# OxfordML/GPz

Measured on AMD Instinct MI355X. Metric: objective+gradient evals/sec, higher is better.
Workload: dtype f64

## Files before the change

### gpz_amd/csrc/gpz_options.h

```cpp
#pragma once

struct gpz_options {
    bool no_graph = false;
    bool graph_debug = false;
    long row_tile = 0;
    long cache_cap_mb = -1;
    bool psi32_mfma = false;
    long predict_min_rows_per_block = 4096;
    bool f32_contractions_off = false;
    bool gc_minv_off = false;
    bool gc_dense_phi_off = false;
    bool tgemm_no_split = false;
    bool phi_diag_no_split = false;
    bool pmc_scratch = false;
    bool pmc_prep_scratch = false;
    bool pmc_no_model_cache = false;
    bool round_phi32 = false;
    bool cpsi_off = false;
    bool cpsi4_off = false;
    bool tgemm_int8 = false;
    int syrk_wgs = 0, syrk_s1 = 0, syrk_s2 = 0;
    int mom_nc = 0;
    int small_stagger = 0;
    bool chol_rowinv_off = false;
    bool syrk_small_off = false;
    bool small_tail_off = false;
    int debug_fail_cut = 0;
};

gpz_options gpz_options_load();

const gpz_options &gpz_opts();
struct gpz_opts_scope {
    const gpz_options *prev;
    explicit gpz_opts_scope(const gpz_options *o);
    ~gpz_opts_scope();
    gpz_opts_scope(const gpz_opts_scope &) = delete;
    gpz_opts_scope &operator=(const gpz_opts_scope &) = delete;
};
```

### gpz_amd/csrc/gpz_options.hip

```cpp
#include <stdlib.h>
#include "gpz_options.h"

static const char *env(const char *name) { return getenv(name); }
static bool env_set(const char *name) { return env(name) != nullptr; }
static long env_long(const char *name, long dflt) {
    const char *e = env(name);
    return e ? atol(e) : dflt;
}

gpz_options gpz_options_load() {
    gpz_options o;
    o.no_graph = env_set("GPZ_NO_GRAPH");
    o.graph_debug = env_set("GPZ_GRAPH_DEBUG");
    o.row_tile = env_long("GPZ_ROW_TILE", 0);
    o.cache_cap_mb = env_long("GPZ_CACHE_CAP_MB", -1);
    {
        const char *e = env("GPZ_PSI32_MFMA");
        o.psi32_mfma = e && e[0] == '1';
    }
    o.predict_min_rows_per_block = env_long("GPZ_PREDICT_MIN_ROWS_PER_BLOCK", 4096);
    if (o.predict_min_rows_per_block < 1) o.predict_min_rows_per_block = 1;
#ifdef GPZ_DEV_SWITCHES
    o.f32_contractions_off = env_set("GPZ_F32_CONTRACTIONS_OFF");
    o.gc_minv_off = env_set("GPZ_GC_MINV_OFF");
    o.gc_dense_phi_off = env_set("GPZ_GC_DENSE_PHI_OFF");
    o.tgemm_no_split = env_set("GPZ_TGEMM_NO_SPLIT");
    o.phi_diag_no_split = env_set("GPZ_PHI_DIAG_NO_SPLIT");
    o.pmc_scratch = env_set("GPZ_PMC_SCRATCH");
    o.pmc_prep_scratch = env_set("GPZ_PMC_PREP_SCRATCH");
    o.pmc_no_model_cache = env_set("GPZ_PMC_NO_MODEL_CACHE");
    o.round_phi32 = env_set("GPZ_EXPERIMENT_ROUND_PHI32");
    o.cpsi_off = env_set("GPZ_CPSI_OFF");
    o.cpsi4_off = env_set("GPZ_CPSI4_OFF");
    o.tgemm_int8 = env_set("GPZ_TGEMM_INT8");
    o.syrk_wgs = (int)env_long("GPZ_SYRK_WGS", 0);
    o.syrk_s1 = (int)env_long("GPZ_SYRK_S1", 0);
    o.syrk_s2 = (int)env_long("GPZ_SYRK_S2", 0);
    o.mom_nc = (int)env_long("GPZ_MOM_NC", 0);
    o.debug_fail_cut = (int)env_long("GPZ_DEBUG_FAIL_CUT", 0);
    o.small_tail_off = env_set("GPZ_SMALL_TAIL_OFF");
    o.syrk_small_off = env_set("GPZ_SYRK_SMALL_OFF");
    o.chol_rowinv_off = env_set("GPZ_CHOL_ROWINV_OFF");
    o.small_stagger = (int)env_long("GPZ_SMALL_STAGGER", 0);
#endif
    return o;
}

static thread_local const gpz_options *t_opts = nullptr;
const gpz_options &gpz_opts() {
    if (t_opts) return *t_opts;
    static const gpz_options process = gpz_options_load();
    return process;
}
gpz_opts_scope::gpz_opts_scope(const gpz_options *o) : prev(t_opts) { t_opts = o; }
gpz_opts_scope::~gpz_opts_scope() { t_opts = prev; }
```

### gpz_amd/csrc/k_gemm.hip

```cpp
#include <type_traits>
#include "gpz_dev.h"
#include "gpz_kernels.h"

#ifdef GPZ_GEMM_TRACE
__device__ unsigned long long *g_gemm_trace = nullptr;
#define GPZ_TRACE_MARK(slot)                                                                                              \
    do {                                                                                                                  \
        if (g_gemm_trace && (threadIdx.x & 63) == 0)                                                                      \
            g_gemm_trace[((size_t)item * 8 + (threadIdx.x >> 6)) * 6 + (slot)] = __builtin_amdgcn_s_memtime();       \
    } while (0)
#else
#define GPZ_TRACE_MARK(slot) do { } while (0)
#endif
typedef float f4_t __attribute__((ext_vector_type(4)));
typedef float f2_t __attribute__((ext_vector_type(2)));
#ifndef GPZ_F32_FLUSH
#define GPZ_F32_FLUSH 8
#endif
template <typename OT> struct MfmaOf;
template <> struct MfmaOf<double> {
    typedef d4_t acc_t;
    typedef d2_t pair_t;
    static __device__ __forceinline__ acc_t run(double a, double b, acc_t c) { return MFMA_F64(a, b, c); }
};
template <> struct MfmaOf<float> {
    typedef f4_t acc_t;
    typedef f2_t pair_t;
    static __device__ __forceinline__ acc_t run(float a, float b, acc_t c) { return __builtin_amdgcn_mfma_f32_16x16x4f32(a, b, c, 0, 0, 0); }
};
template <typename OT>
__device__ __forceinline__ typename MfmaOf<OT>::pair_t to_pair(const f2_t v) {
    typename MfmaOf<OT>::pair_t r;
    r.x = (OT)v.x;
    r.y = (OT)v.y;
    return r;
}
template <typename BT> struct Pair2 { typedef d2_t t; };
template <> struct Pair2<float> { typedef f2_t t; };
template <typename OT>
__device__ __forceinline__ typename MfmaOf<OT>::pair_t to_pair(const d2_t v) {
    typename MfmaOf<OT>::pair_t r;
    r.x = (OT)v.x;
    r.y = (OT)v.y;
    return r;
}

template <bool WEIGHTED, int WC, bool DIAGT, typename OT>
__device__ __forceinline__ void syrk_body(const double *__restrict__ Phi, int ld, const double *__restrict__ wgt,
                                          int mp, int i0, int j0, int r_begin, int r_end,
                                          double *__restrict__ out, OT (*sA)[16][LDS_LD128],
                                          OT (*sB)[16][LDS_LD128], OT (*sW)[16]) {
    constexpr int NT = 128 * WC;
    constexpr int NI = 8 / WC;
    constexpr int Q = 1024 / NT;
    constexpr bool diag_tile = DIAGT;
    constexpr bool PRESCALE = WEIGHTED;
    const int tid = threadIdx.x, lane = tid & 63, wave = tid >> 6;
    const int wr = wave / WC, wc = wave % WC;

    constexpr bool F32 = std::is_same<OT, float>::value;
    typedef typename MfmaOf<OT>::acc_t acc_t;
    typedef typename MfmaOf<OT>::pair_t pair_t;
    acc_t acc[4][NI];
    d4_t acc64[F32 ? 4 : 1][F32 ? NI : 1];
#pragma unroll
    for (int a = 0; a < 4; ++a)
#pragma unroll
        for (int b = 0; b < NI; ++b) {
            acc[a][b] = (acc_t){0, 0, 0, 0};
            if (F32) acc64[a][b] = (d4_t){0.0, 0.0, 0.0, 0.0};
        }
    auto flush = [&]() {
        if constexpr (F32) {
#pragma unroll
            for (int a = 0; a < 4; ++a)
#pragma unroll
                for (int b = 0; b < NI; ++b) {
#pragma unroll
                    for (int r = 0; r < 4; ++r) acc64[a][b][r] += (double)acc[a][b][r];
                    acc[a][b] = (acc_t){0, 0, 0, 0};
                }
        }
    };

    d2_t ra[Q], rb[Q];
    double rw = 0.0, rwq[PRESCALE ? Q : 1];
    const int ca = min(i0 + (tid & 63) * 2, mp - 2), cb = min(j0 + (tid & 63) * 2, mp - 2);
    const unsigned voa = (unsigned)(((tid >> 6) * ld + ca) * 8), vob = (unsigned)(((tid >> 6) * ld + cb) * 8);
    const unsigned vow = (unsigned)((PRESCALE ? (tid >> 6) : (tid & 15)) * 8);
    const size_t qsp = (size_t)(NT / 64) * ld * 8, ksp = (size_t)16 * ld * 8;
    const char *pp = reinterpret_cast<const char *>(Phi + (size_t)r_begin * ld);
    const char *pw = reinterpret_cast<const char *>(WEIGHTED ? wgt + r_begin : nullptr);
    auto gload = [&]() {
        unsigned oa = voa, ob = vob, ow = vow;
        asm volatile("" : "+v"(oa), "+v"(ob), "+v"(ow));
#pragma unroll
        for (int q = 0; q < Q; ++q) {
            ra[q] = *reinterpret_cast<const d2_t *>(pp + q * qsp + oa);
            if (!diag_tile) rb[q] = *reinterpret_cast<const d2_t *>(pp + q * qsp + ob);
            if (PRESCALE) rwq[q] = *reinterpret_cast<const double *>(pw + q * (NT / 64) * 8 + ow);
        }
        if (WEIGHTED && !PRESCALE && tid < 16) rw = *reinterpret_cast<const double *>(pw + ow);
        pp += ksp;
        if (WEIGHTED) pw += 16 * 8;
    };
    auto lstore = [&](int buf) {
#pragma unroll
        for (int q = 0; q < Q; ++q) {
            int idx = q * NT + tid;
            int row = idx >> 6, c = (idx & 63) * 2;
            if (diag_tile) *reinterpret_cast<pair_t *>(&sB[buf][row][c]) = to_pair<OT>(ra[q]);
            else *reinterpret_cast<pair_t *>(&sB[buf][row][c]) = to_pair<OT>(rb[q]);
            if (PRESCALE) { ra[q].x *= rwq[q]; ra[q].y *= rwq[q]; }
            *reinterpret_cast<pair_t *>(&sA[buf][row][c]) = to_pair<OT>(ra[q]);
        }
        if (WEIGHTED && !PRESCALE && tid < 16) sW[buf][tid] = (OT)rw;
    };

    const int nstage = (r_end > r_begin) ? (r_end - r_begin) / 16 : 0;
    if (nstage > 0) {
        gload();
        lstore(0);
        if (nstage > 1) gload();
    }
    __syncthreads();
    static_assert(!DIAGT || NI == 2, "diagonal-tile wave roles are written for the 2 x 4 wave grid");
    constexpr int NA = 4, NB = DIAGT ? 5 : NI;
    int dra[5] = {0, 0, 0, 0, 0}, dcb[5] = {0, 0, 0, 0, 0};
    bool has5 = false;
    if (DIAGT) {
        const int wv = __builtin_amdgcn_readfirstlane(wave);
        const unsigned RA[8] = {0x00000u, 0x11111u, 0x22222u, 0x33333u, 0x77000u, 0x66611u, 0x55552u, 0x44444u};
        const unsigned CB[8] = {0x43210u, 0x54321u, 0x65432u, 0x76543u, 0x77765u, 0x77676u, 0x77657u, 0x77654u};
        has5 = wv < 4;
#pragma unroll
        for (int p = 0; p < 5; ++p) {
            dra[p] = (RA[wv] >> (4 * p)) & 15;
            dcb[p] = (CB[wv] >> (4 * p)) & 15;
        }
    }
    auto rdfrag = [&](int cur, int kk, OT (&a)[NA], OT (&b)[NB]) {
        const OT(*tA)[LDS_LD128] = sA[cur];
        const OT(*tB)[LDS_LD128] = sB[cur];
        const int krow = kk * 4 + (lane >> 4);
        if (DIAGT) {
#pragma unroll
            for (int p = 0; p < 4; ++p) a[p] = tA[krow][dra[p] * 16 + (lane & 15)];
#pragma unroll
            for (int p = 0; p < 5; ++p) b[p] = tB[krow][dcb[p] * 16 + (lane & 15)];
        } else {
#pragma unroll
            for (int mi = 0; mi < 4; ++mi) a[mi] = tA[krow][wr * 64 + mi * 16 + (lane & 15)];
#pragma unroll
            for (int ni = 0; ni < NI; ++ni) b[ni] = tB[krow][wc * (16 * NI) + ni * 16 + (lane & 15)];
        }
    };
    auto burst = [&](const OT (&a)[NA], const OT (&b)[NB]) {
        __builtin_amdgcn_s_setprio(1);
        if (DIAGT) {
#pragma unroll
            for (int p = 0; p < 4; ++p) acc[p][0] = MfmaOf<OT>::run(a[p], b[p], acc[p][0]);
            if (has5) acc[0][1] = MfmaOf<OT>::run(a[0], b[DIAGT ? 4 : 0], acc[0][1]);
        } else {
#pragma unroll
            for (int mi = 0; mi < 4; ++mi)
#pragma unroll
                for (int ni = 0; ni < NI; ++ni) acc[mi][ni] = MfmaOf<OT>::run(a[mi], b[ni], acc[mi][ni]);
        }
        __builtin_amdgcn_s_setprio(0);
    };
    OT fa0[NA] = {}, fb0[NB] = {}, fa1[NA] = {}, fb1[NB] = {};
    if (nstage > 0) rdfrag(0, 0, fa0, fb0);
    auto stage = [&](auto curc, int s) {
        constexpr int cur = decltype(curc)::value;
        rdfrag(cur, 1, fa1, fb1);
        __builtin_amdgcn_sched_barrier(0);
        burst(fa0, fb0);
        __builtin_amdgcn_sched_barrier(0);
        rdfrag(cur, 2, fa0, fb0);
        __builtin_amdgcn_sched_barrier(0);
        burst(fa1, fb1);
        __builtin_amdgcn_sched_barrier(0);
        if (s + 1 < nstage) {
            lstore(cur ^ 1);
            if (s + 2 < nstage) gload();
        }
        rdfrag(cur, 3, fa1, fb1);
        __builtin_amdgcn_sched_barrier(0);
        burst(fa0, fb0);
        __builtin_amdgcn_sched_barrier(0);
        __syncthreads();
        if (s + 1 < nstage) rdfrag(cur ^ 1, 0, fa0, fb0);
        __builtin_amdgcn_sched_barrier(0);
        burst(fa1, fb1);
        __builtin_amdgcn_sched_barrier(0);
    };
    int s = 0;
    for (; s + 1 < nstage; s += 2) {
        stage(std::integral_constant<int, 0>{}, s);
        stage(std::integral_constant<int, 1>{}, s + 1);
        if (F32 && ((s + 2) % GPZ_F32_FLUSH) == 0) flush();
    }
    if (s < nstage) stage(std::integral_constant<int, 0>{}, s);
    flush();
    auto res = [&](int mi, int ni, int r) -> double {
        if constexpr (F32) return acc64[mi][ni][r];
        else return acc[mi][ni][r];
    };
    auto crow = [&](int r) -> int { return F32 ? 4 * (lane >> 4) + r : (lane >> 4) + 4 * r; };

    if (DIAGT) {
#pragma unroll
        for (int p = 0; p < 5; ++p) {
            if (p == 4 && !has5) break;
            const int col = j0 + dcb[p] * 16 + (lane & 15);
#pragma unroll
            for (int r = 0; r < 4; ++r) {
                const int row = i0 + dra[p] * 16 + crow(r);
                if (row < mp && col < mp) out[(size_t)row * mp + col] = p < 4 ? res(p, 0, r) : res(0, 1, r);
            }
        }
    } else {
#pragma unroll
        for (int mi = 0; mi < 4; ++mi)
#pragma unroll
            for (int ni = 0; ni < NI; ++ni) {
                const int col = j0 + wc * (16 * NI) + ni * 16 + (lane & 15);
#pragma unroll
                for (int r = 0; r < 4; ++r) {
                    const int row = i0 + wr * 64 + mi * 16 + crow(r);
                    if (row < mp && col < mp) out[(size_t)row * mp + col] = res(mi, ni, r);
                }
            }
    }
}

template <bool WEIGHTED, bool TRI, int WC, typename OT>
__global__ __launch_bounds__(128 * WC, (std::is_same<OT, float>::value ? 2 : WC)) void k_syrk(
    const double *__restrict__ Phi, int ld, const double *__restrict__ wgt, int n_rows, int mp, int ntile, int nsplit,
    int rows_per_split, int nsplit_d, int rows_per_split_d, double *__restrict__ slab) {
    __shared__ OT sA[2][16][LDS_LD128];
    __shared__ OT sB[2][16][LDS_LD128];
    __shared__ OT sW[2][16];

    const int npairs = ntile * (ntile + 1) / 2;
    const int nwg = gridDim.x, xcd = blockIdx.x & 7, qq = nwg >> 3, rr = nwg & 7;
    const int lb = (xcd < rr ? xcd * (qq + 1) : rr * (qq + 1) + (xcd - rr) * qq) + (blockIdx.x >> 3);
    const int noff = npairs - ntile, ndiag = ntile * nsplit_d;
    auto gstart = [&](int g) { return g * noff + g * ndiag / nsplit; };
    int g = (int)((unsigned)lb * (unsigned)nsplit / (unsigned)(noff * nsplit + ndiag));
    g = g > nsplit - 1 ? nsplit - 1 : g;
    while (g > 0 && gstart(g) > lb) --g;
    while (g + 1 < nsplit && gstart(g + 1) <= lb) ++g;
    const int within = lb - gstart(g);
    int ti, tj, split, rps;
    if (within < noff) {
        split = g;
        rps = rows_per_split;
        int rem = within;
        ti = 0;
        while (rem >= ntile - 1 - ti) { rem -= ntile - 1 - ti; ++ti; }
        tj = ti + 1 + rem;
    } else {
        const int q = g * ndiag / nsplit + within - noff;
        split = q / ntile;
        rps = rows_per_split_d;
        ti = tj = q % ntile;
    }
    const bool diag_tile = (ti == tj);
    const int i0 = ti * 128, j0 = tj * 128;

    int r_begin = split * rps;
    int r_end = min(n_rows, r_begin + rps);
    if (TRI) r_begin = max(r_begin, j0 & ~15);
    double *out = slab + (size_t)split * mp * mp;
    if (diag_tile)
        syrk_body<WEIGHTED, WC, true, OT>(Phi, ld, wgt, mp, i0, j0, r_begin, r_end, out, sA, sB, sW);
    else
        syrk_body<WEIGHTED, WC, false, OT>(Phi, ld, wgt, mp, i0, j0, r_begin, r_end, out, sA, sB, sW);
}

__global__ void k_syrk_reduce(const double *__restrict__ slab, int nsplit_off, int nsplit_d, int mp,
                              double *__restrict__ S, int lds, int accumulate) {
    const int j = blockIdx.x * blockDim.x + threadIdx.x;
    const int i = blockIdx.y;
    if (j >= mp || i > j) return;
    const int ti = i >> 7, tj = j >> 7;
    const int nsplit = (ti == tj) ? nsplit_d : nsplit_off;
    const size_t stride = (size_t)mp * mp;
    const double *p = slab + (size_t)i * mp + j;
    double s0 = 0.0, s1 = 0.0, s2 = 0.0, s3 = 0.0;
    int k = 0;
    for (; k + 8 <= nsplit; k += 8) {
        double v[8];
#pragma unroll
        for (int q = 0; q < 8; ++q) v[q] = p[(size_t)(k + q) * stride];
        s0 += v[0]; s1 += v[1]; s2 += v[2]; s3 += v[3];
        s0 += v[4]; s1 += v[5]; s2 += v[6]; s3 += v[7];
    }
    for (; k < nsplit; ++k) s0 += p[(size_t)k * stride];
    const double t = (s0 + s1) + (s2 + s3);
    S[(size_t)i * lds + j] = accumulate ? S[(size_t)i * lds + j] + t : t;
    if (i != j) S[(size_t)j * lds + i] = accumulate ? S[(size_t)j * lds + i] + t : t;
}

template <bool EDGE, int WC, typename OT, typename BT>
__device__ __forceinline__ void tgemm_body(const double *__restrict__ Phi, int ld, const BT *__restrict__ B,
                                           int ldb, double *__restrict__ T, int ldt, int mp, int i0, int j0,
                                           OT (*sA)[128][18], OT (*sB)[16][LDS_LD128],
                                           double *__restrict__ nupart, double *__restrict__ phiw, int m, int mcol,
                                           long n_pad, int ct, int kdim, int ncol16 = 8, int slot = 0, int nslot = 1, int item = 0) {
    constexpr int NT = 128 * WC;
    constexpr int NI = 8 / WC;
    constexpr int Q = 1024 / NT;
    const int tid = threadIdx.x, lane = tid & 63, wave = tid >> 6;
    const int wr = wave / WC, wc = wave % WC;

    typedef typename MfmaOf<OT>::acc_t acc_t;
    typedef typename MfmaOf<OT>::pair_t pair_t;
    acc_t acc[4][NI];
#pragma unroll
    for (int a = 0; a < 4; ++a)
#pragma unroll
        for (int b = 0; b < NI; ++b) acc[a][b] = (acc_t){0, 0, 0, 0};

    typedef typename Pair2<BT>::t bpair_t;
    d2_t ra[Q];
    bpair_t rb[Q];
    const unsigned voa = (unsigned)(((tid >> 3) * ld + (tid & 7) * 2) * 8);
    const unsigned vob = (unsigned)(((tid >> 6) * ldb + min(j0 + (tid & 63) * 2, mp - 2)) * sizeof(BT));
    const size_t qsa = (size_t)(NT / 8) * ld * 8, qsb = (size_t)(NT / 64) * ldb * sizeof(BT), ksb = (size_t)16 * ldb * sizeof(BT);
    const char *pa = reinterpret_cast<const char *>(Phi + (size_t)i0 * ld);
    const char *pb = reinterpret_cast<const char *>(B);
    auto gload = [&]() {
        unsigned oa = voa, ob = vob;
        asm volatile("" : "+v"(oa), "+v"(ob));
#pragma unroll
        for (int q = 0; q < Q; ++q) {
            ra[q] = *reinterpret_cast<const d2_t *>(pa + q * qsa + oa);
            rb[q] = *reinterpret_cast<const bpair_t *>(pb + q * qsb + ob);
        }
        pa += 16 * 8;
        pb += ksb;
    };
    auto lstore = [&](int buf) {
#pragma unroll
        for (int q = 0; q < Q; ++q) {
            int idx = q * NT + tid;
            int arow = idx >> 3, ac = (idx & 7) * 2;
            *reinterpret_cast<pair_t *>(&sA[buf][arow][ac]) = to_pair<OT>(ra[q]);
            int row = idx >> 6, c = (idx & 63) * 2;
            *reinterpret_cast<pair_t *>(&sB[buf][row][c]) = to_pair<OT>(rb[q]);
        }
    };

    int nvalid = NI;
    if (EDGE) {
        nvalid = (mp - j0 + 15) / 16;
        nvalid = nvalid < 0 ? 0 : (nvalid > ncol16 ? ncol16 : nvalid);
        nvalid = __builtin_amdgcn_readfirstlane(nvalid);
    }
    static_assert(!EDGE || 4 * NI == 8, "the row-strip deal keeps its eight accumulators in acc[4][2]");
    constexpr int NFA = EDGE ? 1 : 4, NFB = EDGE ? 8 : NI;

    const int nstage = kdim / 16;
    gload();
    lstore(0);
    if (nstage > 1) gload();
    __syncthreads();
    auto rdfrag = [&](int cur, int kk, OT (&a)[NFA], OT (&b)[NFB]) {
        const int kc = kk * 4 + (lane >> 4);
        if (EDGE) {
            a[0] = sA[cur][wave * 16 + (lane & 15)][kc];
#pragma unroll
            for (int p = 0; p < NFB; ++p) b[p] = sB[cur][kc][p * 16 + (lane & 15)];
        } else {
#pragma unroll
            for (int mi = 0; mi < NFA; ++mi) a[mi] = sA[cur][wr * 64 + mi * 16 + (lane & 15)][kc];
#pragma unroll
            for (int ni = 0; ni < NI; ++ni) b[ni] = sB[cur][kc][wc * (16 * NI) + ni * 16 + (lane & 15)];
        }
    };
    auto burst = [&](const OT (&a)[NFA], const OT (&b)[NFB]) {
        __builtin_amdgcn_s_setprio(1);
        if (EDGE) {
#pragma unroll
            for (int p = 0; p < NFB; ++p)
                if (p < nvalid) acc[p >> 1][p & 1] = MfmaOf<OT>::run(a[0], b[p], acc[p >> 1][p & 1]);
        } else {
#pragma unroll
            for (int ni = 0; ni < NI; ++ni) {
#pragma unroll
                for (int mi = 0; mi < NFA; ++mi) acc[mi][ni] = MfmaOf<OT>::run(a[mi], b[ni], acc[mi][ni]);
            }
        }
        __builtin_amdgcn_s_setprio(0);
    };
    OT fa0[NFA], fb0[NFB], fa1[NFA], fb1[NFB];
    rdfrag(0, 0, fa0, fb0);
    GPZ_TRACE_MARK(1);
    auto stage = [&](auto curc, int s) {
        constexpr int cur = decltype(curc)::value;
        rdfrag(cur, 1, fa1, fb1);
        __builtin_amdgcn_sched_barrier(0);
        burst(fa0, fb0);
        __builtin_amdgcn_sched_barrier(0);
        rdfrag(cur, 2, fa0, fb0);
        __builtin_amdgcn_sched_barrier(0);
        burst(fa1, fb1);
        __builtin_amdgcn_sched_barrier(0);
        if (s + 1 < nstage) {
            lstore(cur ^ 1);
            if (s + 2 < nstage) gload();
        }
        rdfrag(cur, 3, fa1, fb1);
        __builtin_amdgcn_sched_barrier(0);
        burst(fa0, fb0);
        __builtin_amdgcn_sched_barrier(0);
        __syncthreads();
        if (s + 1 < nstage) rdfrag(cur ^ 1, 0, fa0, fb0);
        __builtin_amdgcn_sched_barrier(0);
        burst(fa1, fb1);
        __builtin_amdgcn_sched_barrier(0);
    };
    int s = 0;
    for (; s + 1 < nstage; s += 2) {
        stage(std::integral_constant<int, 0>{}, s);
        stage(std::integral_constant<int, 1>{}, s + 1);
    }
    if (s < nstage) stage(std::integral_constant<int, 0>{}, s);
    GPZ_TRACE_MARK(2);
    auto res = [&](int mi, int ni, int r) -> double { return (double)acc[mi][ni][r]; };
    auto crow = [&](int r) -> int { return std::is_same<OT, float>::value ? 4 * (lane >> 4) + r : (lane >> 4) + 4 * r; };

    if (EDGE) {
#pragma unroll
        for (int p = 0; p < NFB; ++p) {
            const int col = j0 + p * 16 + (lane & 15);
            if (p < nvalid && col < mp) {
#pragma unroll
                for (int r = 0; r < 4; ++r) T[(size_t)(i0 + wave * 16 + crow(r)) * ldt + col] = res(p >> 1, p & 1, r);
            }
        }
        if (nupart) {
#pragma unroll
            for (int r = 0; r < 4; ++r) {
                const int row = i0 + wave * 16 + crow(r);
                double pp = 0.0;
#pragma unroll
                for (int p = 0; p < NFB; ++p) {
                    const int col = j0 + p * 16 + (lane & 15);
                    if (p < nvalid && col < m) pp = fma(Phi[(size_t)row * ld + col], res(p >> 1, p & 1, r), pp);
                    if (p < nvalid && col == mcol) phiw[row] = res(p >> 1, p & 1, r);
                }
                pp += __shfl_xor(pp, 1, 64);
                pp += __shfl_xor(pp, 2, 64);
                pp += __shfl_xor(pp, 4, 64);
                pp += __shfl_xor(pp, 8, 64);
                if ((lane & 15) == 0) {
                    nupart[(size_t)(ct * WC + slot) * n_pad + row] = pp;
                    if (slot == 0)
#pragma unroll
                        for (int q = 1; q < WC; ++q)
                            if (q >= nslot) nupart[(size_t)(ct * WC + q) * n_pad + row] = 0.0;
                }
            }
        }
        return;
    }
    const int wv = __builtin_amdgcn_readfirstlane(wave);
    const int wru = wv / WC, wcu = wv % WC;
    const char *pbase = reinterpret_cast<const char *>(Phi + (size_t)(i0 + wru * 64) * ld + j0 + wcu * (16 * NI));
    char *tbase = reinterpret_cast<char *>(T + (size_t)(i0 + wru * 64) * ldt + j0 + wcu * (16 * NI));
    double *slotp = nupart ? nupart + (size_t)(ct * WC + wc) * n_pad : nullptr;
#pragma unroll
    for (int hf = 0; hf < 2; ++hf) {
        double ph[2][4][NI];
        if (nupart) {
#pragma unroll
            for (int mh = 0; mh < 2; ++mh)
#pragma unroll
                for (int r = 0; r < 4; ++r)
#pragma unroll
                    for (int ni = 0; ni < NI; ++ni)
                        ph[mh][r][ni] = *reinterpret_cast<const double *>(pbase + ((size_t)((hf * 2 + mh) * 16 + crow(r)) * ld + ni * 16 + (lane & 15)) * 8);
        }
        __builtin_amdgcn_sched_barrier(0);
#pragma unroll
        for (int mh = 0; mh < 2; ++mh)
#pragma unroll
            for (int ni = 0; ni < NI; ++ni) {
#pragma unroll
                for (int r = 0; r < 4; ++r)
                    *reinterpret_cast<double *>(tbase + ((size_t)((hf * 2 + mh) * 16 + crow(r)) * ldt + ni * 16 + (lane & 15)) * 8) = res(hf * 2 + mh, ni, r);
            }
        __builtin_amdgcn_sched_barrier(0);
        if (nupart) {
#pragma unroll
            for (int mh = 0; mh < 2; ++mh)
#pragma unroll
                for (int r = 0; r < 4; ++r) {
                    const int mi = hf * 2 + mh;
                    const int row = i0 + wr * 64 + mi * 16 + crow(r);
                    double p = 0.0;
#pragma unroll
                    for (int ni = 0; ni < NI; ++ni) {
                        const int col = j0 + wc * (16 * NI) + ni * 16 + (lane & 15);
                        const double t = fma(ph[mh][r][ni], res(mi, ni, r), p);
                        p = (col < m) ? t : p;
                        if (col == mcol) phiw[row] = res(mi, ni, r);
                    }
                    p += __shfl_xor(p, 1, 64);
                    p += __shfl_xor(p, 2, 64);
                    p += __shfl_xor(p, 4, 64);
                    p += __shfl_xor(p, 8, 64);
                    if ((lane & 15) == 0) slotp[row] = p;
                }
        }
        __builtin_amdgcn_sched_barrier(0);
    }
}

template <int WC, typename OT, typename BT>
__global__ __launch_bounds__(128 * WC, WC) void k_tgemm(const double *__restrict__ Phi, int ld,
                                                        const BT *__restrict__ B, int ldb,
                                                        double *__restrict__ T, int ldt, int mp, int nct,
                                                        double *__restrict__ nupart, double *__restrict__ phiw, int m,
                                                        int mcol, long n_pad, int kdim, int nfull, int npiece) {
    __shared__ OT sA[2][128][18];
    __shared__ OT sB[2][16][LDS_LD128];
    const int item = blockIdx.x;
#ifdef GPZ_GEMM_TRACE
    GPZ_TRACE_MARK(0);
    if (g_gemm_trace && (threadIdx.x & 63) == 0)
        g_gemm_trace[((size_t)item * 8 + (threadIdx.x >> 6)) * 6 + 4] =
            ((unsigned long long)__builtin_amdgcn_s_getreg((31 << 11) | 20) << 32) | __builtin_amdgcn_s_getreg((31 << 11) | 4);
    struct TraceEnd { int item; __device__ ~TraceEnd() { GPZ_TRACE_MARK(3); } } trace_end{item};
#endif
    if (item >= nfull) {
        const int q = item - nfull;
        const int tile = nfull + q / npiece, piece = q % npiece;
        const int rt = tile / nct, ct = tile % nct;
        tgemm_body<true, WC, OT, BT>(Phi, ld, B, ldb, T, ldt, mp, rt * 128, ct * 128 + piece * (128 / npiece), sA, sB, nupart, phiw, m, mcol,
                                 n_pad, ct, kdim, 8 / npiece, piece, npiece, item);
        return;
    }
    const int nwg = nfull, xcd = item & 7, q = nwg >> 3, r = nwg & 7;
    const int lb = (xcd < r ? xcd * (q + 1) : r * (q + 1) + (xcd - r) * q) + (item >> 3);
    const int rt = lb / nct, ct = lb % nct;
    const int i0 = rt * 128, j0 = ct * 128;
    if (j0 + 128 <= mp)
        tgemm_body<false, WC, OT, BT>(Phi, ld, B, ldb, T, ldt, mp, i0, j0, sA, sB, nupart, phiw, m, mcol, n_pad, ct, kdim, 8, 0, 1, item);
    else
        tgemm_body<true, WC, OT, BT>(Phi, ld, B, ldb, T, ldt, mp, i0, j0, sA, sB, nupart, phiw, m, mcol, n_pad, ct, kdim, 8, 0, 1, item);
}

__device__ void gemm_tile_64(const double *__restrict__ A, long lda, const double *__restrict__ B, long ldb,
                             double *__restrict__ C, long ldc, int M, int N, int kbeg, int kend, double alpha, int tm,
                             int tn) {
    __shared__ double sA[2][16][LDS_LD64];
    __shared__ double sB[2][16][LDS_LD64];
    const int tid = threadIdx.x, lane = tid & 63, wave = tid >> 6;
    const int wr = wave >> 1, wc = wave & 1;
    const int i0 = tm * 64, j0 = tn * 64;
    d4_t acc[2][2];
#pragma unroll
    for (int a = 0; a < 2; ++a)
#pragma unroll
        for (int b = 0; b < 2; ++b) acc[a][b] = (d4_t){0.0, 0.0, 0.0, 0.0};

    const int ar = tid >> 2, ak = (tid & 3) * 4;
    const int bk = tid >> 4, bc = (tid & 15) * 4;
    const bool aok = i0 + ar < M, bok = j0 + bc < N;
    const double *ap = A + (size_t)(i0 + ar) * lda + ak;
    const double *bp = B + (size_t)bk * ldb + j0 + bc;
    struct Regs { d2_t a[2], b[2]; } r0, r1;
    auto gload = [&](Regs &r, int k0) {
        const d2_t z = {0.0, 0.0};
        r.a[0] = aok ? *reinterpret_cast<const d2_t *>(ap + k0) : z;
        r.a[1] = aok ? *reinterpret_cast<const d2_t *>(ap + k0 + 2) : z;
        r.b[0] = bok ? *reinterpret_cast<const d2_t *>(bp + (size_t)k0 * ldb) : z;
        r.b[1] = bok ? *reinterpret_cast<const d2_t *>(bp + (size_t)k0 * ldb + 2) : z;
    };
    auto park = [&](const Regs &r, int buf) {
        sA[buf][ak + 0][ar] = r.a[0][0]; sA[buf][ak + 1][ar] = r.a[0][1]; sA[buf][ak + 2][ar] = r.a[1][0]; sA[buf][ak + 3][ar] = r.a[1][1];
        *reinterpret_cast<d2_t *>(&sB[buf][bk][bc]) = r.b[0];
        *reinterpret_cast<d2_t *>(&sB[buf][bk][bc + 2]) = r.b[1];
    };
    auto multiply = [&](int buf) {
#pragma unroll
        for (int kk = 0; kk < 4; ++kk) {
            const int kr = kk * 4 + (lane >> 4);
            double a[2], b[2];
#pragma unroll
            for (int mi = 0; mi < 2; ++mi) a[mi] = sA[buf][kr][wr * 32 + mi * 16 + (lane & 15)];
#pragma unroll
            for (int ni = 0; ni < 2; ++ni) b[ni] = sB[buf][kr][wc * 32 + ni * 16 + (lane & 15)];
#pragma unroll
            for (int mi = 0; mi < 2; ++mi)
#pragma unroll
                for (int ni = 0; ni < 2; ++ni) acc[mi][ni] = MFMA_F64(a[mi], b[ni], acc[mi][ni]);
        }
    };
    if (kbeg < kend) {
        gload(r0, kbeg);
        if (kbeg + 16 < kend) gload(r1, kbeg + 16);
        park(r0, 0);
        __syncthreads();
    }
    for (int k0 = kbeg; k0 < kend; k0 += 32) {
        if (k0 + 32 < kend) gload(r0, k0 + 32);
        multiply(0);
        if (k0 + 16 >= kend) break;
        park(r1, 1);
        __syncthreads();
        if (k0 + 48 < kend) gload(r1, k0 + 48);
        multiply(1);
        if (k0 + 32 < kend) park(r0, 0);
        __syncthreads();
    }
#pragma unroll
    for (int mi = 0; mi < 2; ++mi)
#pragma unroll
        for (int ni = 0; ni < 2; ++ni) {
            const int col = j0 + wc * 32 + ni * 16 + (lane & 15);
#pragma unroll
            for (int r = 0; r < 4; ++r) {
                const int row = i0 + wr * 32 + mi * 16 + (lane >> 4) + 4 * r;
                if (row < M && col < N) C[row * ldc + col] = alpha * acc[mi][ni][r];
            }
        }
}

__global__ __launch_bounds__(256) void k_trtri_level(const double *__restrict__ L, double *__restrict__ W,
                                                      double *__restrict__ Tmp, int ld, int mq, int gs, int phase) {
    const int p = blockIdx.z;
    const int a = p * 2 * gs;
    const int rb = a + gs;
    if (rb >= mq) return;
    const int Mr = min(gs, mq - rb);
    const int tm = blockIdx.y, tn = blockIdx.x;
    if (tm * 64 >= Mr) return;
    if (phase == 0) {
        gemm_tile_64(L + (size_t)rb * ld + a, ld, W + (size_t)a * ld + a, ld, Tmp + (size_t)rb * ld + a, ld, Mr, gs,
                     tn * 64, gs, 1.0, tm, tn);
    } else {
        gemm_tile_64(W + (size_t)rb * ld + rb, ld, Tmp + (size_t)rb * ld + a, ld, W + (size_t)rb * ld + a, ld, Mr, gs,
                     0, min(Mr, tm * 64 + 64), -1.0, tm, tn);
    }
}

#ifndef GPZ_GEMM_WC
#define GPZ_GEMM_WC 4
#endif
int gpz_gemm_wave_cols() { return GPZ_GEMM_WC; }

void launch_syrk(hipStream_t st, const double *Phi, int ld, const double *wgt, int n_rows, int mp,
                 int nsplit, int rows_per_split, int nsplit_d, int rows_per_split_d, double *slab, bool tri,
                 bool f32_operands) {
    constexpr int WC = GPZ_GEMM_WC;
    const int ntile = (mp + 127) / 128;
    const int noff = ntile * (ntile - 1) / 2;
    dim3 grid(noff * nsplit + ntile * nsplit_d), block(128 * WC);
    if (tri)
        hipLaunchKernelGGL((k_syrk<false, true, WC, double>), grid, block, 0, st, Phi, ld, wgt, n_rows, mp, ntile, nsplit,
                           rows_per_split, nsplit_d, rows_per_split_d, slab);
    else if (wgt && f32_operands)
        hipLaunchKernelGGL((k_syrk<true, false, WC, float>), grid, block, 0, st, Phi, ld, wgt, n_rows, mp, ntile, nsplit,
                           rows_per_split, nsplit_d, rows_per_split_d, slab);
    else if (wgt)
        hipLaunchKernelGGL((k_syrk<true, false, WC, double>), grid, block, 0, st, Phi, ld, wgt, n_rows, mp, ntile, nsplit,
                           rows_per_split, nsplit_d, rows_per_split_d, slab);
    else
        hipLaunchKernelGGL((k_syrk<false, false, WC, double>), grid, block, 0, st, Phi, ld, wgt, n_rows, mp, ntile, nsplit,
                           rows_per_split, nsplit_d, rows_per_split_d, slab);
}

void launch_syrk_reduce(hipStream_t st, const double *slab, int nsplit, int nsplit_d, int mp, double *S, int lds, int accumulate) {
    dim3 block(256), grid((mp + 255) / 256, mp);
    hipLaunchKernelGGL(k_syrk_reduce, grid, block, 0, st, slab, nsplit, nsplit_d, mp, S, lds, accumulate);
}

int gpz_cu_count() {
    static const int n = [] {
        int dev = 0, cu = 0;
        if (hipGetDevice(&dev) != hipSuccess || hipDeviceGetAttribute(&cu, hipDeviceAttributeMultiprocessorCount, dev) != hipSuccess || cu <= 0) cu = 256;
        return cu;
    }();
    return n;
}

__global__ void k_round_f32(const double *__restrict__ src, float *__restrict__ dst, size_t n) {
    const size_t i = (size_t)blockIdx.x * blockDim.x + threadIdx.x;
    if (i < n) dst[i] = (float)src[i];
}
void launch_round_f32(hipStream_t st, const double *src, float *dst, size_t n) {
    hipLaunchKernelGGL(k_round_f32, dim3((unsigned)((n + 255) / 256)), dim3(256), 0, st, src, dst, n);
}

void launch_tgemm(hipStream_t st, const double *Phi, int ld, const double *B, int ldb, double *T, int n_pad, int mp,
                  double *nupart, double *phiw, int m, int mcol, bool f32_operands, int kdim, int ldt, const float *B32) {
    constexpr int WC = GPZ_GEMM_WC;
    const int nct = (mp + 127) / 128;
    if (kdim <= 0) kdim = mp;
    if (ldt <= 0) ldt = ld;
    const int W = (n_pad / 128) * nct, C = 2 * gpz_cu_count();
    int tail = W % C, npiece = 1;
    const bool no_split = gpz_opts().tgemm_no_split;
    if (tail > 0 && !no_split && tail * 4 <= C) npiece = 4;
    if (npiece == 1) tail = 0;
    const int nfull = W - tail;
    dim3 grid(nfull + tail * npiece), block(128 * WC);
    if (f32_operands && B32)
        hipLaunchKernelGGL((k_tgemm<WC, float, float>), grid, block, 0, st, Phi, ld, B32, ldb, T, ldt, mp, nct, nupart, phiw, m, mcol,
                           (long)n_pad, kdim, nfull, npiece);
    else if (f32_operands)
        hipLaunchKernelGGL((k_tgemm<WC, float, double>), grid, block, 0, st, Phi, ld, B, ldb, T, ldt, mp, nct, nupart, phiw, m, mcol,
                           (long)n_pad, kdim, nfull, npiece);
    else
        hipLaunchKernelGGL((k_tgemm<WC, double, double>), grid, block, 0, st, Phi, ld, B, ldb, T, ldt, mp, nct, nupart, phiw, m, mcol,
                           (long)n_pad, kdim, nfull, npiece);
}

void launch_trtri_level(hipStream_t st, const double *L, double *W, double *Tmp, int ld, int mq, int gs) {
    const int npair = (mq + 2 * gs - 1) / (2 * gs);
    const int nt = (gs + 63) / 64;
    hipLaunchKernelGGL(k_trtri_level, dim3(nt, nt, npair), dim3(256), 0, st, L, W, Tmp, ld, mq, gs, 0);
    hipLaunchKernelGGL(k_trtri_level, dim3(nt, nt, npair), dim3(256), 0, st, L, W, Tmp, ld, mq, gs, 1);
}
```

Before: 18.27.

## Stage fp64 tgemm tiles into LDS via global_load_lds DMA with swizzled layout

Adds an LDS-DMA path for the fp64 tgemm kernel. It uses global_load_lds_dwordx4 to copy A and B tiles straight from global memory into shared memory, bypassing register staging and the separate LDS store. The A tile drops its padding and uses an XOR swizzle for fragment reads, and the next stage is issued mid-loop followed by a vmcnt wait before the barrier. The old register-staging path stays behind an env switch; the new path relies on inline asm and M0 handling, and adds a full vmcnt wait each stage.

Result: faster. 18.50 (median of 6 runs) (+1.2%).

```diff
diff --git a/gpz_amd/csrc/gpz_options.h b/gpz_amd/csrc/gpz_options.h
--- a/gpz_amd/csrc/gpz_options.h
+++ b/gpz_amd/csrc/gpz_options.h
@@ -11,6 +11,7 @@
     bool gc_minv_off = false;
     bool gc_dense_phi_off = false;
     bool tgemm_no_split = false;
+    bool gemm_reg_staging = false;
     bool phi_diag_no_split = false;
     bool pmc_scratch = false;
     bool pmc_prep_scratch = false;
diff --git a/gpz_amd/csrc/gpz_options.hip b/gpz_amd/csrc/gpz_options.hip
--- a/gpz_amd/csrc/gpz_options.hip
+++ b/gpz_amd/csrc/gpz_options.hip
@@ -25,6 +25,7 @@
     o.gc_minv_off = env_set("GPZ_GC_MINV_OFF");
     o.gc_dense_phi_off = env_set("GPZ_GC_DENSE_PHI_OFF");
     o.tgemm_no_split = env_set("GPZ_TGEMM_NO_SPLIT");
+    o.gemm_reg_staging = env_set("GPZ_GEMM_REG_STAGING");
     o.phi_diag_no_split = env_set("GPZ_PHI_DIAG_NO_SPLIT");
     o.pmc_scratch = env_set("GPZ_PMC_SCRATCH");
     o.pmc_prep_scratch = env_set("GPZ_PMC_PREP_SCRATCH");
diff --git a/gpz_amd/csrc/k_gemm.hip b/gpz_amd/csrc/k_gemm.hip
--- a/gpz_amd/csrc/k_gemm.hip
+++ b/gpz_amd/csrc/k_gemm.hip
@@ -12,6 +12,12 @@
 #else
 #define GPZ_TRACE_MARK(slot) do { } while (0)
 #endif
+__device__ __forceinline__ void gemm_glds(const void *base, unsigned voff, const void *lds) {
+    const unsigned l = (unsigned)(uintptr_t)(const __attribute__((address_space(3))) void *)lds;
+    unsigned keep;
+    asm volatile("s_mov_b32 %0, m0\n\ts_mov_b32 m0, %3\n\ts_nop 0\n\tglobal_load_lds_dwordx4 %1, %2\n\ts_mov_b32 m0, %0"
+                 : "=&s"(keep) : "v"(voff), "s"(base), "s"(l) : "memory");
+}
 typedef float f4_t __attribute__((ext_vector_type(4)));
 typedef float f2_t __attribute__((ext_vector_type(2)));
 #ifndef GPZ_F32_FLUSH
@@ -304,10 +310,10 @@
     if (i != j) S[(size_t)j * lds + i] = accumulate ? S[(size_t)j * lds + i] + t : t;
 }
 
-template <bool EDGE, int WC, typename OT, typename BT>
+template <bool EDGE, int WC, typename OT, typename BT, bool DMA, int AL>
 __device__ __forceinline__ void tgemm_body(const double *__restrict__ Phi, int ld, const BT *__restrict__ B,
                                            int ldb, double *__restrict__ T, int ldt, int mp, int i0, int j0,
-                                           OT (*sA)[128][18], OT (*sB)[16][LDS_LD128],
+                                           OT (*sA)[128][AL], OT (*sB)[16][LDS_LD128],
                                            double *__restrict__ nupart, double *__restrict__ phiw, int m, int mcol,
                                            long n_pad, int ct, int kdim, int ncol16 = 8, int slot = 0, int nslot = 1, int item = 0) {
     constexpr int NT = 128 * WC;
@@ -353,6 +359,30 @@
             *reinterpret_cast<pair_t *>(&sB[buf][row][c]) = to_pair<OT>(rb[q]);
         }
     };
+    static_assert(!DMA || (std::is_same<OT, double>::value && std::is_same<BT, double>::value && AL == 16), "LDS-DMA staging: fp64 operands");
+    static_assert(DMA || AL == 18, "register staging: padded A rows");
+    const int wvu = __builtin_amdgcn_readfirstlane(wave);
+    const unsigned dsw = 4u * (unsigned)(wvu & 1) + (unsigned)(lane >> 4);
+    const unsigned doa = (unsigned)(((8 * wvu + (lane >> 3)) * ld + 2 * (int)((unsigned)(lane & 7) ^ dsw)) * 8);
+    const unsigned dob = (unsigned)((wvu * ldb + min(j0 + lane * 2, mp - 2)) * 8);
+    const size_t da64 = (size_t)64 * ld * 8, db8 = (size_t)8 * ldb * sizeof(BT);
+    auto dma = [&](int buf) {
+        OT *la = &sA[buf][8 * wvu][0];
+        OT *lb = &sB[buf][wvu][0];
+        gemm_glds(pa, doa, la);
+        gemm_glds(pa + da64, doa, la + 64 * AL);
+        gemm_glds(pb, dob, lb);
+        gemm_glds(pb + db8, dob, lb + 8 * LDS_LD128);
+        pa += 16 * 8;
+        pb += ksb;
+    };
+    int adx[4] = {0, 0, 0, 0};
+    if constexpr (DMA) {
+        const int r0 = EDGE ? wave * 16 : wr * 64;
+#pragma unroll
+        for (int kk = 0; kk < 4; ++kk)
+            adx[kk] = (r0 + (lane & 15)) * AL + 2 * (((2 * kk) | (lane >> 5)) ^ ((lane >> 1) & 7)) + ((lane >> 4) & 1);
+    }
 
     int nvalid = NI;
     if (EDGE) {
@@ -364,13 +394,29 @@
     constexpr int NFA = EDGE ? 1 : 4, NFB = EDGE ? 8 : NI;
 
     const int nstage = kdim / 16;
-    gload();
-    lstore(0);
-    if (nstage > 1) gload();
+    if constexpr (DMA) {
+        dma(0);
+        asm volatile("s_waitcnt vmcnt(0)" ::: "memory");
+    } else {
+        gload();
+        lstore(0);
+        if (nstage > 1) gload();
+    }
     __syncthreads();
     auto rdfrag = [&](int cur, int kk, OT (&a)[NFA], OT (&b)[NFB]) {
         const int kc = kk * 4 + (lane >> 4);
-        if (EDGE) {
+        if constexpr (DMA) {
+            const OT *tA = &sA[cur][0][0];
+#pragma unroll
+            for (int mi = 0; mi < NFA; ++mi) a[mi] = tA[adx[kk] + mi * 16 * AL];
+            if (EDGE) {
+#pragma unroll
+                for (int p = 0; p < NFB; ++p) b[p] = sB[cur][kc][p * 16 + (lane & 15)];
+            } else {
+#pragma unroll
+                for (int ni = 0; ni < NI; ++ni) b[ni] = sB[cur][kc][wc * (16 * NI) + ni * 16 + (lane & 15)];
+            }
+        } else if (EDGE) {
             a[0] = sA[cur][wave * 16 + (lane & 15)][kc];
 #pragma unroll
             for (int p = 0; p < NFB; ++p) b[p] = sB[cur][kc][p * 16 + (lane & 15)];
@@ -405,11 +451,13 @@
         __builtin_amdgcn_sched_barrier(0);
         burst(fa0, fb0);
         __builtin_amdgcn_sched_barrier(0);
+        if (DMA && s + 1 < nstage) dma(cur ^ 1);
+        __builtin_amdgcn_sched_barrier(0);
         rdfrag(cur, 2, fa0, fb0);
         __builtin_amdgcn_sched_barrier(0);
         burst(fa1, fb1);
         __builtin_amdgcn_sched_barrier(0);
-        if (s + 1 < nstage) {
+        if (!DMA && s + 1 < nstage) {
             lstore(cur ^ 1);
             if (s + 2 < nstage) gload();
         }
@@ -417,6 +465,7 @@
         __builtin_amdgcn_sched_barrier(0);
         burst(fa0, fb0);
         __builtin_amdgcn_sched_barrier(0);
+        if (DMA) asm volatile("s_waitcnt vmcnt(0)" ::: "memory");
         __syncthreads();
         if (s + 1 < nstage) rdfrag(cur ^ 1, 0, fa0, fb0);
         __builtin_amdgcn_sched_barrier(0);
@@ -521,13 +570,13 @@
     }
 }
 
-template <int WC, typename OT, typename BT>
+template <int WC, typename OT, typename BT, bool DMA>
 __global__ __launch_bounds__(128 * WC, WC) void k_tgemm(const double *__restrict__ Phi, int ld,
                                                         const BT *__restrict__ B, int ldb,
                                                         double *__restrict__ T, int ldt, int mp, int nct,
                                                         double *__restrict__ nupart, double *__restrict__ phiw, int m,
                                                         int mcol, long n_pad, int kdim, int nfull, int npiece) {
-    __shared__ OT sA[2][128][18];
+    __shared__ OT sA[2][128][DMA ? 16 : 18];
     __shared__ OT sB[2][16][LDS_LD128];
     const int item = blockIdx.x;
 #ifdef GPZ_GEMM_TRACE
@@ -541,7 +590,7 @@
         const int q = item - nfull;
         const int tile = nfull + q / npiece, piece = q % npiece;
         const int rt = tile / nct, ct = tile % nct;
-        tgemm_body<true, WC, OT, BT>(Phi, ld, B, ldb, T, ldt, mp, rt * 128, ct * 128 + piece * (128 / npiece), sA, sB, nupart, phiw, m, mcol,
+        tgemm_body<true, WC, OT, BT, DMA>(Phi, ld, B, ldb, T, ldt, mp, rt * 128, ct * 128 + piece * (128 / npiece), sA, sB, nupart, phiw, m, mcol,
                                  n_pad, ct, kdim, 8 / npiece, piece, npiece, item);
         return;
     }
@@ -550,9 +599,9 @@
     const int rt = lb / nct, ct = lb % nct;
     const int i0 = rt * 128, j0 = ct * 128;
     if (j0 + 128 <= mp)
-        tgemm_body<false, WC, OT, BT>(Phi, ld, B, ldb, T, ldt, mp, i0, j0, sA, sB, nupart, phiw, m, mcol, n_pad, ct, kdim, 8, 0, 1, item);
+        tgemm_body<false, WC, OT, BT, DMA>(Phi, ld, B, ldb, T, ldt, mp, i0, j0, sA, sB, nupart, phiw, m, mcol, n_pad, ct, kdim, 8, 0, 1, item);
     else
-        tgemm_body<true, WC, OT, BT>(Phi, ld, B, ldb, T, ldt, mp, i0, j0, sA, sB, nupart, phiw, m, mcol, n_pad, ct, kdim, 8, 0, 1, item);
+        tgemm_body<true, WC, OT, BT, DMA>(Phi, ld, B, ldb, T, ldt, mp, i0, j0, sA, sB, nupart, phiw, m, mcol, n_pad, ct, kdim, 8, 0, 1, item);
 }
 
 __device__ void gemm_tile_64(const double *__restrict__ A, long lda, const double *__restrict__ B, long ldb,
@@ -712,13 +761,16 @@
     const int nfull = W - tail;
     dim3 grid(nfull + tail * npiece), block(128 * WC);
     if (f32_operands && B32)
-        hipLaunchKernelGGL((k_tgemm<WC, float, float>), grid, block, 0, st, Phi, ld, B32, ldb, T, ldt, mp, nct, nupart, phiw, m, mcol,
+        hipLaunchKernelGGL((k_tgemm<WC, float, float, false>), grid, block, 0, st, Phi, ld, B32, ldb, T, ldt, mp, nct, nupart, phiw, m, mcol,
                            (long)n_pad, kdim, nfull, npiece);
     else if (f32_operands)
-        hipLaunchKernelGGL((k_tgemm<WC, float, double>), grid, block, 0, st, Phi, ld, B, ldb, T, ldt, mp, nct, nupart, phiw, m, mcol,
+        hipLaunchKernelGGL((k_tgemm<WC, float, double, false>), grid, block, 0, st, Phi, ld, B, ldb, T, ldt, mp, nct, nupart, phiw, m, mcol,
+                           (long)n_pad, kdim, nfull, npiece);
+    else if (gpz_opts().gemm_reg_staging)
+        hipLaunchKernelGGL((k_tgemm<WC, double, double, false>), grid, block, 0, st, Phi, ld, B, ldb, T, ldt, mp, nct, nupart, phiw, m, mcol,
                            (long)n_pad, kdim, nfull, npiece);
     else
-        hipLaunchKernelGGL((k_tgemm<WC, double, double>), grid, block, 0, st, Phi, ld, B, ldb, T, ldt, mp, nct, nupart, phiw, m, mcol,
+        hipLaunchKernelGGL((k_tgemm<WC, double, double, true>), grid, block, 0, st, Phi, ld, B, ldb, T, ldt, mp, nct, nupart, phiw, m, mcol,
                            (long)n_pad, kdim, nfull, npiece);
 }
 
```
